# nanoshimarobot/dynamic_direct_lidar_odometry

Measured on AMD Instinct MI355X. Metric: GICP iters/sec + ms/scan, 131k-pt source → 500k-pt submap; pose Δ vs CPU ref, higher is better.
Workload: dtype f32 search / f64 normal equations; 1 GPU; cfg3 S2M GICP: 131,072-pt 64x2048 scan -> 500,000-pt 4-keyframe submap, LM, maxCorr 2.0 m, maxIter 32, transEps 0.01; target_points=500000, parallelism=replicas x1

## Files before the change

dynamic_direct_lidar_odometry_amd/__init__.py:

```python
from __future__ import annotations

import ctypes as C
import math
import os
import sys

import numpy as np

__all__ = ["GicpParams", "GicpResult", "Context", "NanoGICP", "GicpError", "lib_path", "load", "s2s_batch",
           "REG_NONE", "REG_MIN_EIG", "REG_NORMALIZED_MIN_EIG", "REG_PLANE", "REG_FROBENIUS",
           "GAUSS_NEWTON", "LEVENBERG_MARQUARDT", "SOURCE", "TARGET"]

REG_NONE, REG_MIN_EIG, REG_NORMALIZED_MIN_EIG, REG_PLANE, REG_FROBENIUS = range(5)
GAUSS_NEWTON, LEVENBERG_MARQUARDT = 0, 1
SOURCE, TARGET = 0, 1
COV_MAT4D, COV_SYM6 = 0, 1

_HERE = os.path.dirname(os.path.abspath(__file__))
_LIB = None

STATUS = {0: "GICP_OK", 1: "GICP_EINVAL", 2: "GICP_ENOTARGET", 3: "GICP_ENOSOURCE", 4: "GICP_ETOOFEW",
          5: "GICP_EHIP", 6: "GICP_ENOMEM", 7: "GICP_ESTATE", 8: "GICP_ENONFINITE", 9: "GICP_ECOMM"}


# ... 153 lines not shown
        "gicp_get_tie_order": (I, [P, C.POINTER(C.c_int)]),
        "gicp_set_option": (I, [P, I, I]),
        "gicp_get_option": (I, [P, I, C.POINTER(C.c_int)]),
        "gicp_set_default_option": (I, [I, I]),
        "gicp_get_default_option": (I, [I, C.POINTER(C.c_int)]),
        "gicp_tie_builder_set": (I, [P, P, C.c_size_t, C.c_size_t]),
        "gicp_tie_builder_export": (I, [P, P, C.c_size_t, C.POINTER(C.c_void_p), C.POINTER(C.c_size_t)]),
        "gicp_set_tie_tree": (I, [P, P, C.c_size_t]),
        "gicp_set_tie_trees_from_root": (I, [P, I, P, P]),
        "gicp_get_device_bytes": (I, [P, C.POINTER(C.c_int64), I]),
        "gicp_debug_nftree": (I, [P, I, P, P, P, S, C.POINTER(S)]),
        "gicp_debug_nfbuild": (I, [P, I, I, P, P, P, P, S]),
        "gicp_set_target_grid": (I, [P, I]),
        "gicp_get_target_grid_info": (I, [P, C.POINTER(GicpGridInfo)]),
        "gicp_get_lookup_stats": (I, [P, C.POINTER(C.c_int64)]),
    }
    for name, (res, args) in sig.items():
        f = getattr(L, name)
        f.restype = res
        f.argtypes = args
    _LIB = L
    return L


def default_params(**kw) -> GicpParams:
    p = GicpParams()
    load().gicp_default_params(C.byref(p))
    for k, v in kw.items():
        setattr(p, k, v)
    return p


def _ptr(a):
# ... 227 lines not shown
        return idx, d

    def set_target_grid(self, mode=GRID_AUTO):
        self._check(self.L.gicp_set_target_grid(self.h, int(mode)))

    def grid_info(self) -> dict:
        info = GicpGridInfo()
        self._check(self.L.gicp_get_target_grid_info(self.h, C.byref(info)))
        return info.as_dict()

    def lookup_walk_groups(self) -> int:
        v = C.c_int64(0)
        self._check(self.L.gicp_get_lookup_stats(self.h, C.byref(v)))
        return int(v.value)

    def set_tie_order(self, nanoflann_order=True):
        self._check(self.L.gicp_set_tie_order(self.h, 1 if nanoflann_order else 0))

    def nftree(self, side):
        nn = C.c_size_t(0)
        self._check(self.L.gicp_debug_nftree(self.h, side, None, None, None, 0, C.byref(nn)))
        n = self.size(side)
        vind = np.empty(n, np.int32)
        nodes = np.empty((nn.value, 4), np.int32)
        div = np.empty((nn.value, 2), np.float32)
        self._check(self.L.gicp_debug_nftree(self.h, side, _ptr(vind), _ptr(nodes), _ptr(div), nn.value, C.byref(nn)))
        return vind, nodes, div

    def nfbuild_debug(self, side, stop=-1, scratch_bytes=1 << 20):
        n = self.size(side)
# ... 184 lines not shown
```

dynamic_direct_lidar_odometry_amd/csrc/capi.hip:

```cpp
#include <hip/hip_runtime.h>

#include <atomic>
#include <thread>

#include <hipcub/hipcub.hpp>
#include <rccl/rccl.h>

#include <dlfcn.h>

#include <algorithm>
#include <cfloat>
#include <cmath>
#include <cstdio>
#include <cstdlib>
#include <cstring>
#include <limits>
#include <map>
#include <memory>
#include <mutex>
#include <string>
#include <tuple>
#include <thread>
#include <vector>

// ... 453 lines not shown
    none->info.build_status = s;
    t.grid = none;
    g_last_error.clear();
    return GICP_OK;
  }
  t.grid = g;
  return GICP_OK;
}

struct JobCommit {
  gicp_ctx* c;
  bool ok = false;
  explicit JobCommit(gicp_ctx* ctx) : c(ctx) {}
  void done() { ok = true; }
  ~JobCommit() {
    if (!ok) c->job_last_valid = false;
  }
};

void finalize_job(gicp_ctx* c) {
  AlignJob& j = *c->job_host;
  j.job_full = 0;
  AlignJob probe = j;
  std::memcpy(probe.guess_R, c->job_last.guess_R, sizeof(probe.guess_R));
  std::memcpy(probe.guess_t, c->job_last.guess_t, sizeof(probe.guess_t));
  probe.job_full = c->job_last.job_full;
  probe.ticket = c->job_last.ticket;
  if (!c->job_last_valid || std::memcmp(&probe, &c->job_last, sizeof(AlignJob)) != 0) {
    j.job_full = 1;
    c->job_last = j;
    c->job_last_valid = true;
// ... 208 lines not shown
void drop_set(GraphSet& gs) {
  for (auto& p : gs.first) drop_pair(p);
  gs.first.clear();
  drop_pair(gs.rest[0]);
  drop_pair(gs.rest[1]);
  gs.key.fill(-1);
}

void drop_graphs(gicp_ctx* c) {
  for (auto& gs : c->gsets) drop_set(gs);
  c->gsets.clear();
}

gicp_status graph_set(gicp_ctx* c, const std::array<long long, 7>& key, int nblocks, GraphSet** out);

gicp_status run_align_graph(gicp_ctx* c, int max_it, int nblocks, int* final_chunk) {
  const void* jd = c->job_dev.p;
  const LinGeom g = geometry(c);
  (void)nblocks;
  const std::array<long long, 7> key{{(long long)(uintptr_t)c->slab.p | (c->comm ? 1 : 0), (long long)(uintptr_t)jd,
                                      g.seed_blocks, g.scan_blocks, g.mom_blocks, g.lds_boxes,
                                      g.grid ? (g.grid_walk ? 2L : 1L) * g.lookup_blocks : 0}};
  const bool use_graph = !c->comm || c->comm_graphs;
  const int first = c->params.fixed_iterations > 0
                        ? std::max(1, std::min(max_it, kMaxFixedChunk))
                        : std::max(1, std::min({c->predicted_iters, max_it, kMaxFirstChunk}));
  GraphSet* gs = nullptr;
  if (use_graph) {
    gicp_status s = graph_set(c, key, nblocks, &gs);
    if (s) {
      drop_graphs(c);
      (void)hipGetLastError();
      if (!c->comm) return s;
      c->comm_graphs = false;
      return run_align_graph(c, max_it, nblocks, final_chunk);
    }
  }
  if (use_graph && !gs->first[first - 1].ge) {
    gicp_status s = capture_chunk(c, true, first, nblocks, 0, &gs->first[first - 1]);
    if (s) {
      drop_graphs(c);
      return s;
    }
  }
  auto launch_chunk = [&](int k) -> gicp_status {
    const bool is_first = k == 0;
    if (use_graph) {
      HIP_TRY(hipGraphLaunch(is_first ? gs->first[first - 1].ge : gs->rest[k & 1].ge, c->stream));
      return GICP_OK;
    }
    return enqueue_chunk(c, is_first, is_first ? first : 1, nblocks, k & 1);
  };
  const int nchunks = 1 + (max_it - first);
  while ((int)c->chunk_ev.size() < nchunks) {
    hipEvent_t e;
    HIP_TRY(hipEventCreateWithFlags(&e, hipEventDisableTiming));
    c->chunk_ev.push_back(e);
  }
  gicp_status s = launch_chunk(0);
  if (s) return s;
  HIP_TRY(hipEventRecord(c->chunk_ev[0], c->stream));
// ... 366 lines not shown
  c->tie_tree.reset();
  invalidate_align(c);
  return GICP_OK;
}

gicp_status gicp_share_source(gicp_ctx* dst, const gicp_ctx* src) {
  if (!dst || !src) return fail(GICP_EINVAL, "null ctx");
  if (dst->device != src->device) return fail(GICP_EINVAL, "contexts live on different devices");
  dst->src = src->src;
  invalidate_align(dst);
  return GICP_OK;
}

gicp_status gicp_align(gicp_ctx* c, const float* guess16, float* out16, gicp_result* res) {
  if (!c) return fail(GICP_EINVAL, "null ctx");
  begin_ties(c);
  gicp_status s = set_device(c);
  if (s) return s;
  s = maybe_build_grid(c);
  if (s) return s;
  s = prepare_align(c);
  if (s) return s;
  const int ns = c->src.cloud->n;
  const int nblocks = linearize_blocks(ns);
  hipEvent_t end_ev = c->ev1;
  int reruns = 0;
  for (;;) {
    s = fill_job(c, guess16, nblocks);
    if (s) return s;
    finalize_job(c);
    JobCommit commit(c);
    const int max_it = c->job_host->max_iterations;
    end_ev = c->ev1;
    if (c->profiling) HIP_TRY(hipEventRecord(c->ev0, c->stream));
    if (c->profiling || max_it <= 0) {
      s = max_it > 0 ? run_align_eager_profiled(c, max_it, nblocks) : GICP_OK;
      if (s) return s;
      if (max_it <= 0) launch_align_init(c->stream, c->job_dev.as<AlignJob>(), c->job_host_dev);
      HIP_TRY(hipGetLastError());
      commit.done();
      HIP_TRY(hipEventRecord(c->ev1, c->stream));
      HIP_TRY(hipMemcpyAsync(c->state_host, c->state_dev.p, sizeof(AlignState), hipMemcpyDeviceToHost, c->stream));
      HIP_TRY(hipStreamSynchronize(c->stream));
      c->state_slot = 0;
      c->tail_pending = false;
    } else {
      int fc = 0;
      s = run_align_graph(c, max_it, nblocks, &fc);
      if (s) return s;
      commit.done();
      end_ev = c->chunk_ev[fc];
    }
    if (!final_state(c).tie_pending || reruns > 0) break;
    s = ensure_tie_tree(c);
    if (s) return s;
    ++reruns;
  }
  const AlignState& st = final_state(c);
  c->have_align = st.iter > 0;
  c->last_nsrc = ns;
  if (out16) {
    for (int r = 0; r < 3; ++r) {
      for (int cc = 0; cc < 3; ++cc) out16[4 * r + cc] = (float)st.R[3 * r + cc];
      out16[4 * r + 3] = (float)st.t[r];
    }
// ... 21 lines not shown
      double tot = 0.0;
      for (int i = 0; i < st.iter; ++i) {
        float m = 0.f;
        HIP_TRY(hipEventElapsedTime(&m, c->prof_ev[2 * i], c->prof_ev[2 * i + 1]));
        tot += m;
      }
      res->linearize_ms = tot;
    }
  }
  s = check_ties(c);
  if (s) return s;
  if (st.tie_err || st.tie_pending)
    return fail(GICP_EHIP, "nanoflann tie order: a tied correspondence could not be re-run (bits " +
                               std::to_string(st.tie_err) + (st.tie_pending ? ", no tree" : "") + ")");
  if (st.lm_failed) g_last_error = "lm not converged!!";
  return GICP_OK;
}

gicp_status gicp_get_residuals(gicp_ctx* c, double* out, size_t n) {
  if (!c || !out) return fail(GICP_EINVAL, "null argument");
  if (!c->have_align || !c->src.cloud || !c->tgt.cloud) return fail(GICP_ESTATE, "no linearization to report residuals of");
  if ((int)n != c->src.cloud->n) return fail(GICP_EINVAL, "n != source size");
  gicp_status s = set_device(c);
  if (s) return s;
  HIP_TRY(c->tmp_out.ensure(sizeof(double) * n));
  launch_residuals(c->stream, c->job_dev.as<AlignJob>(), (int)n, c->tmp_out.as<double>());
  HIP_TRY(hipGetLastError());
  if (c->comm)
    NCCL_TRY(rccl().all_reduce(c->tmp_out.p, c->tmp_out.p, n, ncclFloat64, ncclMin, c->comm, c->stream));
  HIP_TRY(hipMemcpyAsync(out, c->tmp_out.p, sizeof(double) * n, hipMemcpyDeviceToHost, c->stream));
// ... 66 lines not shown
  const size_t bytes = (n - 1) * stride + 12;
  HIP_TRY(c->tmp_out.ensure(bytes + 256));
  float* dT = reinterpret_cast<float*>(c->tmp_out.as<char>() + ((bytes + 63) / 64) * 64);
  HIP_TRY(hipMemcpyAsync(dT, T, sizeof(T), hipMemcpyHostToDevice, c->stream));
  HIP_TRY(hipMemcpyAsync(c->tmp_out.p, out_xyz, bytes, hipMemcpyHostToDevice, c->stream));
  launch_transform(c->stream, c->src.cloud->pts.as<float4>(), (int)n, c->src.cloud->perm.as<int>(), dT,
                   c->tmp_out.as<float>(), stride / 4);
  HIP_TRY(hipGetLastError());
  HIP_TRY(hipMemcpyAsync(out_xyz, c->tmp_out.p, bytes, hipMemcpyDeviceToHost, c->stream));
  HIP_TRY(hipStreamSynchronize(c->stream));
  return GICP_OK;
}

gicp_status gicp_linearize(gicp_ctx* c, const double* pose16, double* H36, double* b6, double* cost, int32_t* ncorr) {
  if (!c || !pose16) return fail(GICP_EINVAL, "null argument");
  begin_ties(c);
  gicp_status s = set_device(c);
  if (s) return s;
  s = maybe_build_grid(c);
  if (s) return s;
  s = prepare_align(c);
  if (s) return s;
  const int ns = c->src.cloud->n;
  const int nblocks = linearize_blocks(ns);
  for (int rerun = 0;; ++rerun) {
    float g[16];
    for (int i = 0; i < 16; ++i) g[i] = 0.f;
    s = fill_job(c, g, nblocks);
    if (s) return s;
    for (int r = 0; r < 3; ++r) {
// ... 167 lines not shown
}

gicp_status gicp_set_target_grid(gicp_ctx* c, int mode) {
  if (!c) return fail(GICP_EINVAL, "null ctx");
  if (mode < GICP_GRID_OFF || mode > GICP_GRID_ON) return fail(GICP_EINVAL, "grid mode must be 0 (off), 1 (auto) or 2 (on)");
  c->grid_mode = mode;
  return GICP_OK;
}

gicp_status gicp_get_target_grid_info(gicp_ctx* c, gicp_grid_info* out) {
  if (!c || !out) return fail(GICP_EINVAL, "null argument");
  std::memset(out, 0, sizeof(*out));
  if (!c->tgt.cloud || !c->tgt.cloud->grid) return GICP_OK;
  *out = c->tgt.cloud->grid->info;
  out->built = grid_active(c) ? 1 : 0;
  return GICP_OK;
}

gicp_status gicp_get_lookup_stats(gicp_ctx* c, int64_t* walk_groups) {
  if (!c || !walk_groups) return fail(GICP_EINVAL, "null argument");
  *walk_groups = -1;
  if (!c->fb.p || !c->src.cloud) return GICP_OK;
  gicp_status s = set_device(c);
  if (s) return s;
  unsigned v = 0;
  const FbLayout fl(c->src.cloud->n);
  HIP_TRY(hipMemcpyAsync(&v, c->fb.as<char>() + fl.ctr + sizeof(unsigned) * kFbSegs * 32, sizeof(unsigned),
                         hipMemcpyDeviceToHost, c->stream));
  HIP_TRY(hipStreamSynchronize(c->stream));
  *walk_groups = v;
// ... 580 lines not shown
```

dynamic_direct_lidar_odometry_amd/csrc/gicp_types.hpp:

```cpp
#pragma once
#include <stdint.h>

namespace ddlo {

constexpr int kLeafSize = 32;
constexpr int kFanout = 64;
constexpr int kMaxLevels = 5;
constexpr int kDirBits = 18;
constexpr int kFineBits = 6;
constexpr int kFineMin = 32;
__host__ __device__ constexpr long fine_dir_ints(int n) {
  return (1L << kDirBits) + 2 + (1L << kDirBits) + ((long)(n / (kFineMin + 1) + 1) << kFineBits) / 2;
}

constexpr int kMoments = 74;
constexpr int kMomentSlots = 96;
constexpr int kSlabStride = 80;
constexpr int kStatFields = 8;

constexpr int kTaskRegions = 64;
constexpr int kCtrStride = 32;
constexpr int kTasksPerGroup = 48;

struct CloudDev {
// ... 153 lines not shown
  unsigned long long* key2;
  int tie_detect;
  int tie_ab;
  int tie_scan;
  const int* tgt_nf_status;
  NfTreeDev tgt_nf;
  int grid_on;
  CellGridDev grid;
  unsigned* fb_count;
  int* fb_list;
  int fb_seg_cap;
  unsigned short* fb_mask;
};
constexpr int kFbSegs = 8;

constexpr int kNfMaxLevels = 40;
constexpr int kNfLevelSpare = 2;

struct NfCtl {
  int nnodes, nsmall, err;
  int nchunks[2];
  int ntask[kNfMaxLevels + 1];
  int dbg[16];
};

struct NfTask {
  int node, begin, count, chunk0;
  float lo[3], hi[3];
  unsigned mm[6];
  int feat;
// ... 57 lines not shown
```

dynamic_direct_lidar_odometry_amd/csrc/launch.hpp:

```cpp
#pragma once
#include <hip/hip_runtime.h>

#include "gicp_types.hpp"

namespace ddlo {

void launch_pack_bbox(hipStream_t s, const unsigned char* raw, size_t stride, int n, float4* out, float* partial,
                      int* nonfinite, int nblocks);
void launch_bbox_final(hipStream_t s, const float* partial, int nparts, float* quant);
void launch_morton(hipStream_t s, const float4* pts, int n, const float* quant, unsigned long long* keys, int* vals);
void launch_gather(hipStream_t s, const float4* raw, const int* perm, int n, int npad, float4* sorted, int* inv_perm);
void launch_key_dir(hipStream_t s, const unsigned long long* keys, int n, int* dir);
void launch_leaf_soa_boxes(hipStream_t s, const float4* pts, int n, int nleaves, float* soa, float4* lo, float4* hi);
void launch_level_boxes(hipStream_t s, const float4* clo, const float4* chi, int nchild, int nparent, float4* plo,
                        float4* phi);
struct TieList {
  int* list;
  int* count;
  int cap = 0;
  __device__ __forceinline__ void push(int i) const {
    const int slot = atomicAdd(count, 1);
    if (slot < cap) list[slot] = i;
  }
};
// ... 7 lines not shown
void launch_cov_export(hipStream_t s, const double* cov6, int layout, int n, const int* perm, double* out);
size_t tie_prune_scratch_bytes(int n, int cap);
hipError_t launch_tie_prune(hipStream_t s, const NfTreeDev& t, int cap, const int* local_index, int n_local,
                            void* scratch, NfNode* out_nodes, float4* out_pts, unsigned* counts);
void launch_align_init(hipStream_t s, AlignJob* job, const AlignJob* job_src);
struct LinGeom {
  int seed_blocks, scan_blocks, mom_blocks, lds_boxes, lookup_blocks;
  bool fuse_lm = false;
  AlignState* state = nullptr;
  bool grid = false;
  bool grid_walk = true;
};
bool lm_fusion_enabled(bool lookup);
LinGeom linearize_geometry(int nsrc, int tgt_upper);
void launch_linearize(hipStream_t s, const AlignJob* job, const LinGeom& g, AlignState* publish = nullptr);
int search_queries_per_wave();
int task_cap_per_region(int nsrc);
int moment_blocks(int nsrc);
int lm_slab_rows_max();
void launch_lm_step(hipStream_t s, const AlignJob* job, AlignState* st, const double* slab, int nblocks,
                    const double* premom, AlignState* publish);
void launch_mom_reduce(hipStream_t s, const AlignJob* job);
void launch_residuals(hipStream_t s, const AlignJob* job, int nsrc, double* out);
void launch_residual_image(hipStream_t s, const float4* pts, const int* perm, const int* inv_perm, int n,
                           const double* residual, double tmin, double tmax, int W, int H, int* winner, float* img,
                           float* xyz);
void launch_transform(hipStream_t s, const float4* pts, int n, const int* perm, const float* T16, float* out,
                      size_t stride_floats);
void launch_export_corr(hipStream_t s, const AlignJob* job, int nsrc, int* corr, float* sqd);

// ... 37 lines not shown
```

dynamic_direct_lidar_odometry_amd/csrc/lm_step.hpp:

```cpp
#pragma once
#include <hip/hip_runtime.h>

#include "gicp_types.hpp"
#include "search.hpp"

namespace ddlo {

static __device__ void so3_exp_d(const double w[3], double R[9]) {
  const double theta_sq = w[0] * w[0] + w[1] * w[1] + w[2] * w[2];
  double imag, real;
  if (theta_sq < 1e-10) {
    const double theta_quad = theta_sq * theta_sq;
    imag = 0.5 - 1.0 / 48.0 * theta_sq + 1.0 / 3840.0 * theta_quad;
    real = 1.0 - 1.0 / 8.0 * theta_sq + 1.0 / 384.0 * theta_quad;
  } else {
    const double theta = sqrt(theta_sq);
    const double half = 0.5 * theta;
    double sh, ch;
    sincos(half, &sh, &ch);
    imag = sh / theta;
    real = ch;
  }
  const double qw = real, qx = imag * w[0], qy = imag * w[1], qz = imag * w[2];
  const double tx = 2 * qx, ty = 2 * qy, tz = 2 * qz;
// ... 202 lines not shown
  if (tid < kSlabStride) {
    double s = 0.0;
#pragma unroll
    for (int p = 0; p < kLmParts; ++p) s += part[p][tid];
    mom[tid] = s;
  }
}

#ifdef DDLO_LM_PROF
#define LM_PROF(i) if (threadIdx.x == 0) lm_t[i] = __builtin_amdgcn_s_memtime()
#define LM_PROF_TRIAL(i) if (threadIdx.x == 0) lm_tt[i] = __builtin_amdgcn_s_memtime()
#else
#define LM_PROF(i)
#define LM_PROF_TRIAL(i)
#endif
template <bool PREMOM>
__device__ __forceinline__ void lm_step_body(const AlignJob* __restrict__ job, AlignState* __restrict__ st,
                                             const double* __restrict__ slab, int nblocks,
                                             const double* __restrict__ premom) {
#ifdef DDLO_LM_PROF
  unsigned long long lm_t[6], lm_tt[4] = {0, 0, 0, 0};
#endif
  LM_PROF(0);
  __shared__ double part[kLmParts][kSlabStride];
  __shared__ double mom[kSlabStride];
  __shared__ double nq[kNeqEntries];
  double* const Hs = nq;
  double* const bs = nq + 36;
  double* const W12 = nq + 42;
  double* const g12 = nq + 186;
  __shared__ double tr_lambda[kMaxTrials], tr_cm[kMaxTrials], tr_fro[kMaxTrials];
  __shared__ double tr_R[kMaxTrials][9], tr_t[kMaxTrials][3];
  __shared__ double tr_d[kMaxTrials][12], tr_row[kMaxTrials][12], tr_den[kMaxTrials], tr_x[kMaxTrials][6];
  __shared__ double Rt_s[12];
  __shared__ int tr_conv[kMaxTrials];
  const int tid = threadIdx.x;
  const int it_pre = st->iter;
  const int trials_pre = st->lm_trials;
  const int rec_pre = st->rec;
  const float src_radius = st->src_radius;
  const double lambda_pre = st->lambda;
  double rt_v = 0.0;
  if (tid < 12) rt_v = tid < 9 ? st->R[tid] : st->t[tid - 9];
  const int optimizer = job->optimizer, lm_max_iterations = job->lm_max_iterations;
  const int fixed_iterations = job->fixed_iterations, max_iterations = job->max_iterations;
  const double lm_init_lambda_factor = job->lm_init_lambda_factor;
  const double rotation_epsilon = job->rotation_epsilon, transformation_epsilon = job->transformation_epsilon;
  const int reuse = job->reuse;
  const float reuse_rec_eps = job->reuse_rec_eps, reuse_rec_conv = job->reuse_rec_conv;
  NeqTerm E{};
  if (tid < kNeqEntries) E = kNeq.e[tid];
  if constexpr (PREMOM) {
    if (tid < kSlabStride) mom[tid] = gp(premom)[tid];
  } else {
    reduce_slab(slab, nblocks, part, mom);
  }
  if (tid < 12) Rt_s[tid] = rt_v;
  __syncthreads();
// ... 90 lines not shown
    ok = ball != 0ull;
    chosen = ok ? (int)__builtin_ctzll(ball) : ntr - 1;
    const double rho_c = __shfl(rho, chosen);
    accept = ok && !(rho_c < 0);
    if (lane == 0) {
      st->lm_trials = trials_pre + (ok ? chosen + 1 : ntr);
      if (accept) {
        const double c = 2 * rho_c - 1;
        st->lambda = tr_lambda[chosen] * fmax(1.0 / 3.0, 1 - c * c * c);
      } else if (ok) {
        st->lambda = tr_lambda[chosen];
      } else {
        st->lambda = tr_lambda[ntr - 1] * 2.0;
      }
    }
  }
  if (lane == 0) {
    st->nr_iterations = it_pre;
    st->final_cost = mom[kMomY0];
    st->num_corr = (int)mom[kMomCount];
    if (rec_pre) st->any_rec = 1;
    st->iter = it_pre + 1;
    st->have_prev = 1;
    int done = 0;
    if (!ok) {
      st->lm_failed = 1;
      done = 1;
    } else if (tr_conv[chosen]) {
      st->converged = 1;
      done = 1;
    }
    if (it_pre + 1 >= max_iterations) done = 1;
    if (done) st->done = 1;
  }
  double v = 0.0;
  if (accept) {
    const double* Rd = tr_R[chosen];
    if (lane < 9) {
      const int i = lane / 3, j = lane % 3;
      v = Rd[3 * i + 0] * Rt_s[0 + j] + Rd[3 * i + 1] * Rt_s[3 + j] + Rd[3 * i + 2] * Rt_s[6 + j];
      st->R[lane] = v;
    } else if (lane < 12) {
      const int i = lane - 9;
      v = (Rd[3 * i + 0] * Rt_s[9] + Rd[3 * i + 1] * Rt_s[10] + Rd[3 * i + 2] * Rt_s[11]) + tr_t[chosen][i];
      st->t[i] = v;
    } else if (lane >= 16 && lane < 16 + 36) {
      st->final_hessian[lane - 16] = Hs[lane - 16];
    }
  }
  int rec = reuse;
  if (accept) {
    const double tn0 = __shfl(v, 9), tn1 = __shfl(v, 10), tn2 = __shfl(v, 11);
    const double* dt = tr_t[chosen];
    const double mv = sqrt(tr_fro[chosen]) * ((double)src_radius + sqrt(tn0 * tn0 + tn1 * tn1 + tn2 * tn2)) +
                      sqrt(dt[0] * dt[0] + dt[1] * dt[1] + dt[2] * dt[2]);
    rec = rec && mv < (double)reuse_rec_eps && (fixed_iterations > 0 || tr_cm[chosen] > (double)reuse_rec_conv);
  }
  if (lane == 0) st->rec = rec;
  LM_PROF(5);
#ifdef DDLO_LM_PROF
  if (tid == 0)
    printf("lm_prof %d %llu %llu %llu %llu %llu %llu %llu %llu %llu\n", it_pre, lm_t[1] - lm_t[0], lm_t[2] - lm_t[1],
           lm_t[3] - lm_t[2], lm_t[4] - lm_t[3], lm_t[5] - lm_t[4], lm_tt[0] - lm_t[2], lm_tt[1] - lm_tt[0],
// ... 6 lines not shown
```

dynamic_direct_lidar_odometry_amd/csrc/moments.hip:

```cpp
#include <hip/hip_runtime.h>

#include <cstddef>

#include "gicp_types.hpp"
#include "search.hpp"
#include "nftree.hpp"
#include "cov_math.hpp"
#include "launch.hpp"
#include "launch_util.hpp"
#include "linearize_internal.hpp"
#include "lm_step.hpp"

namespace ddlo {

struct Contrib {
  double M[6];
  double q[3];
  double qq[6];
  double v[3];
  double y;
  double c;
};

template <int S>
// ... 193 lines not shown
  int pending, resolved, err;
};
constexpr int kTieThread = 64 * (kMomWaves - 1);
__device__ __forceinline__ TieWords fetch_tie_words(AlignState* st) {
  TieWords tw{0, 0, 0};
  __hip_atomic_compare_exchange_strong(&st->tie_pending, &tw.pending, 0, __ATOMIC_RELAXED, __ATOMIC_RELAXED,
                                       __HIP_MEMORY_SCOPE_AGENT);
  __hip_atomic_compare_exchange_strong(&st->ties_resolved, &tw.resolved, 0, __ATOMIC_RELAXED, __ATOMIC_RELAXED,
                                       __HIP_MEMORY_SCOPE_AGENT);
  __hip_atomic_compare_exchange_strong(&st->tie_err, &tw.err, 0, __ATOMIC_RELAXED, __ATOMIC_RELAXED,
                                       __HIP_MEMORY_SCOPE_AGENT);
  return tw;
}

__device__ __forceinline__ void publish_state(const AlignJob* __restrict__ job, AlignState* __restrict__ st,
                                              AlignState* __restrict__ publish, const TieWords& tw) {
  static_assert(sizeof(AlignState) % 8 == 0, "AlignState is copied in 8-byte words");
  static_assert(offsetof(AlignState, pub) == sizeof(AlignState) - 8, "the publication word is the last 8 bytes");
  static_assert(offsetof(AlignState, iter) % 8 == 0 && offsetof(AlignState, done) == offsetof(AlignState, iter) + 4,
                "iter and done are one 8-byte word");
  __shared__ int tie_s[3];
  if (threadIdx.x == kTieThread) {
    tie_s[0] = tw.pending;
    tie_s[1] = tw.resolved;
    tie_s[2] = tw.err;
  }
  asm volatile("s_waitcnt vmcnt(0)" ::: "memory");
  __syncthreads();
  const auto src = gpw(reinterpret_cast<unsigned long long*>(st));
  const auto dst = gpw(reinterpret_cast<unsigned long long*>(publish));
  constexpr int kWords = (int)(sizeof(AlignState) / 8);
// ... 1 lines not shown
  auto patch = [](unsigned long long v, int w, size_t off, int val) {
    if ((size_t)w != off / 8) return v;
    const int sh = (int)(off & 4) * 8;
    return (v & ~(0xffffffffull << sh)) | ((unsigned long long)(unsigned)val << sh);
  };
  __shared__ unsigned long long iter_s;
  const int w = threadIdx.x;
  if (w < kWords) {
    unsigned long long v = __hip_atomic_load(src + w, __ATOMIC_RELAXED, __HIP_MEMORY_SCOPE_AGENT);
    v = patch(v, w, offsetof(AlignState, tie_pending), tie_s[0]);
    v = patch(v, w, offsetof(AlignState, ties_resolved), tie_s[1]);
    v = patch(v, w, offsetof(AlignState, tie_err), tie_s[2]);
    dst[w] = v;
    if (w == (int)(offsetof(AlignState, iter) / 8)) iter_s = v;
  }
  const unsigned long long tk = job->ticket;
  asm volatile("s_waitcnt vmcnt(0)" ::: "memory");
  __syncthreads();
  if (threadIdx.x == 0) {
    const unsigned long long id = iter_s;
    const unsigned long long w = (tk << 17) | ((unsigned long long)((unsigned)(id >> 32) != 0u) << 16) | (id & 0xffffu);
    __hip_atomic_store(&publish->pub, w, __ATOMIC_RELEASE, __HIP_MEMORY_SCOPE_SYSTEM);
  }
}

template <bool FUSE_LM, bool LOOKUP = false>
__global__ __launch_bounds__(64 * kMomWaves) void k_moments(const AlignJob* __restrict__ job,
                                                            AlignState* __restrict__ st, AlignState* __restrict__ publish) {
#ifdef DDLO_MOM_PROF
  unsigned long long mp_t[kMomProfWords] = {0, 0, 0, 0, 0, 0, 0};
#endif
  MOM_PROF(0);
  const auto sg = gp(st);
  double R[9], t[3];
  for (int e = 0; e < 9; ++e) R[e] = sg->R[e];
  for (int e = 0; e < 3; ++e) t[e] = sg->t[e];
  const int st_rec = sg->rec, st_any_rec = sg->any_rec;
  if (__builtin_amdgcn_readfirstlane(sg->done)) {
    if (FUSE_LM && publish && blockIdx.x == 0) {
      TieWords tw{};
      if (threadIdx.x == kTieThread) tw = fetch_tie_words(st);
      publish_state(job, st, publish, tw);
    }
    return;
  }
  const CloudDev src = job->src;
  const CloudDev tgt = job->tgt;
  const auto src_cov = gp(job->src_cov);
  const auto tgt_cov = gp(job->tgt_cov);
  const auto key = gp((const unsigned long long*)job->key);
  const auto corr = gpw(job->corr);
  const auto sqd = gpw(job->sqd);
  const auto slab = gpw(job->slab);
  const double max_corr2 = job->max_corr2;
  const int rec = st_rec;
  const int first_rec_done = st_any_rec;
  const int tie_detect = job->tie_detect;
  const bool slice_check = tie_detect && job->tie_scan >= 2 && !(job->tie_ab & 4);
  const bool tie3m = tie_detect && job->tie_scan == 3 && !rec;
  __shared__ NfWaveStack tie_stk[kMomWaves];
  const int lane = lane_id();
  const int wib = threadIdx.x >> 6;
#ifdef DDLO_MOM_PROF
  __builtin_amdgcn_s_waitcnt(0);
#endif
  MOM_PROF(1);
  const int wave = blockIdx.x * kMomWaves + wib;
  const int nwaves_total = gridDim.x * kMomWaves;
  const int ngroups = (src.n + 63) >> 6;
  if (blockIdx.x == 0 && threadIdx.x < kTaskRegions) job->task_ctr[threadIdx.x * kCtrStride] = 0u;
  if (blockIdx.x == 0 && job->grid_on && threadIdx.x == 0) {
    unsigned t = 0;
    for (int sg = 0; sg < kFbSegs; ++sg) t += job->fb_count[sg * 32];
    job->fb_count[kFbSegs * 32] += t;
    for (int sg = 0; sg < kFbSegs; ++sg) job->fb_count[sg * 32] = 0u;
  }
  double acc0 = 0.0, acc1 = 0.0, acc2 = 0.0;
  for (int g = wave; g < ngroups; g += nwaves_total) {
    const int i = g * 64 + lane;
    const bool active = i < src.n;
    int j = -1;
    unsigned kj = 0xffffffffu;
    float kd = INFINITY;
    bool tied = false;
    float4 a = make_float4(0.f, 0.f, 0.f, 0.f), b = a;
    double ca[6] = {0, 0, 0, 0, 0, 0}, cb[6] = {0, 0, 0, 0, 0, 0};
    float lqx = 0.f, lqy = 0.f, lqz = 0.f;
    unsigned long long lkey = 0ull;
    unsigned lsec = 0xffffffffu;
// ... 233 lines not shown
    __shared__ int last_s;
    asm volatile("s_waitcnt vmcnt(0)" ::: "memory");
    __syncthreads();
    unsigned* const arrive = job->task_ctr + kTaskRegions * kCtrStride;
    if (threadIdx.x == 0) last_s = atomicAdd(arrive, 1u) == gridDim.x - 1;
    __syncthreads();
    if (!last_s) return;
    if (threadIdx.x == 0) {
      __builtin_amdgcn_fence(__ATOMIC_ACQUIRE, "agent");
      asm volatile("s_waitcnt vmcnt(0)" ::: "memory");
      atomicExch(arrive, 0u);
    }
    __syncthreads();
    TieWords tw{};
    if (publish && threadIdx.x == kTieThread) tw = fetch_tie_words(st);
    lm_step_body<false>(job, st, job->slab, job->nblocks, nullptr);
    if (publish) publish_state(job, st, publish, tw);
  }
}
template __global__ void k_moments<false>(const AlignJob*, AlignState*, AlignState*);
template __global__ void k_moments<true>(const AlignJob*, AlignState*, AlignState*);
template __global__ void k_moments<false, true>(const AlignJob*, AlignState*, AlignState*);
template __global__ void k_moments<true, true>(const AlignJob*, AlignState*, AlignState*);

__global__ __launch_bounds__(kLmThreads) void k_mom_reduce(const AlignJob* __restrict__ job) {
  AlignState* st = job->state;
  if (__builtin_amdgcn_readfirstlane(st->done)) return;
  __shared__ double part[kLmParts][kSlabStride];
  __shared__ double mom[kSlabStride];
  reduce_slab(job->slab, job->nblocks, part, mom);
  __syncthreads();
  if (threadIdx.x < kSlabStride) gpw(job->mom)[threadIdx.x] = mom[threadIdx.x];
}

__global__ __launch_bounds__(kLmThreads) void k_lm_step(const AlignJob* __restrict__ job, AlignState* __restrict__ st,
                                                        const double* __restrict__ slab, int nblocks,
                                                        const double* __restrict__ premom,
                                                        AlignState* __restrict__ publish) {
  TieWords tw{};
  if (publish && threadIdx.x == kTieThread) tw = fetch_tie_words(st);
  if (!__builtin_amdgcn_readfirstlane(st->done)) {
    if (premom) lm_step_body<true>(job, st, slab, nblocks, premom);
    else lm_step_body<false>(job, st, slab, nblocks, nullptr);
  }
  if (publish) publish_state(job, st, publish, tw);
}

void launch_linearize(hipStream_t s, const AlignJob* job, const LinGeom& g, AlignState* publish) {
  static const int fused_lookup = env_knob("DDLO_GRID_FUSED", 1);
  if (g.grid && !g.grid_walk && fused_lookup) {
    if (g.fuse_lm) k_moments<true, true><<<g.mom_blocks, 64 * kMomWaves, 0, s>>>(job, g.state, publish);
    else k_moments<false, true><<<g.mom_blocks, 64 * kMomWaves, 0, s>>>(job, g.state, nullptr);
    return;
  }
  if (g.grid) launch_cell_lookup(s, job, g);
  if (!g.grid || g.grid_walk) launch_nn_walk(s, job, g);
  if (g.fuse_lm) k_moments<true><<<g.mom_blocks, 64 * kMomWaves, 0, s>>>(job, g.state, publish);
  else k_moments<false><<<g.mom_blocks, 64 * kMomWaves, 0, s>>>(job, g.state, nullptr);
}
int moment_blocks(int nsrc) {
  const int groups = (nsrc + 63) / 64;
  return std::max(1, std::min((groups + kMomWaves - 1) / kMomWaves, kMomBlocksMax));
}
int lm_slab_rows_max() { return kMomBlocksMax; }
void launch_lm_step(hipStream_t s, const AlignJob* job, AlignState* st, const double* slab, int nblocks,
                    const double* premom, AlignState* publish) {
  k_lm_step<<<1, kLmThreads, 0, s>>>(job, st, slab, nblocks, premom, publish);
}
void launch_mom_reduce(hipStream_t s, const AlignJob* job) { k_mom_reduce<<<1, kLmThreads, 0, s>>>(job); }

}

#ifdef DDLO_MOM_PROF
extern "C" int ddlo_dev_mom_prof(unsigned long long* out) {
// ... 4 lines not shown
```

dynamic_direct_lidar_odometry_amd/csrc/runtime.hpp:

```cpp
#pragma once
#include <hip/hip_runtime.h>

#include <hipcub/hipcub.hpp>
#include <rccl/rccl.h>

#include <array>
#include <cfloat>
#include <cmath>
#include <cstring>
#include <map>
#include <memory>
#include <mutex>
#include <string>
#include <tuple>
#include <vector>

#include "../../include/ddlo_gicp.h"
#include "gicp_types.hpp"
#include "launch.hpp"
#include "devknobs.hpp"

#define HIP_TRY(expr)                                                                       \
  do {                                                                                      \
    hipError_t _e = (expr);                                                                 \
// ... 296 lines not shown
constexpr int kNfGraphs = 4;

constexpr int kDefaultPredictedIters = 4;

struct gicp_ctx {
  int device = 0;
  hipStream_t stream = nullptr;
  gicp_params params{};
  Side src, tgt;
  DevBuf raw_bytes, raw_pts, partial, nonfinite, keys_tmp, vals_tmp, sort_tmp, knn;
  DevBuf corr, sqd, slab, job_dev, state_dev, tmp_out, stats;
  bool stats_on = false;
  AlignJob* job_host = nullptr;
  AlignJob job_last{};
  bool job_last_valid = false;
  AlignJob* job_host_dev = nullptr;
  AlignState* state_host_dev = nullptr;
  AlignState* state_host = nullptr;
  int state_slot = 0;
  hipEvent_t tail_ev = nullptr;
  bool tail_pending = false;
  int grid_max_mb = 0;
  unsigned long long ticket = 0;
  int* flag_host = nullptr;
  bool have_align = false;
  int last_nsrc = 0;
  std::vector<GraphSet> gsets;
  long long graph_clock = 0;
  int predicted_iters = kDefaultPredictedIters;
  std::vector<hipEvent_t> chunk_ev;
// ... 532 lines not shown
          for (int p : pos) std::fprintf(f, " %d", p < side.cloud->n ? perm[p] : -1);
          std::fprintf(f, "\n");
          std::fclose(f);
        }
      }
    }
  }
  HIP_TRY(hipGetLastError());
  side.cov = cv;
  return GICP_OK;
}

inline void invalidate_align(gicp_ctx* c) {
  c->have_align = false;
  c->job_last_valid = false;
}

}
}
```

include/ddlo_gicp.h:

```cpp
#ifndef DDLO_GICP_H
#define DDLO_GICP_H

#include <stddef.h>
#include <stdint.h>

#ifdef __cplusplus
extern "C" {
#endif

#define DDLO_GICP_ABI_VERSION 4

typedef enum gicp_status {
  GICP_OK = 0,
  GICP_EINVAL = 1,
  GICP_ENOTARGET = 2,
  GICP_ENOSOURCE = 3,
  GICP_ETOOFEW = 4,
  GICP_EHIP = 5,
  GICP_ENOMEM = 6,
  GICP_ESTATE = 7,
  GICP_ENONFINITE = 8,
  GICP_ECOMM = 9
} gicp_status;

// ... 103 lines not shown
  int64_t bytes;
  int64_t coarse_cells;
  int64_t band_cells;
  int64_t nomatch_cells;
  int64_t overflow_cells;
  int64_t level_cells[4];
  int64_t fine_cells;
  int64_t fallback_fine;
  int64_t entries;
  int64_t uses_walk;
  int64_t build_status;
  int64_t scratch_bytes;
} gicp_grid_info;
gicp_status gicp_get_target_grid_info(struct gicp_ctx* ctx, gicp_grid_info* out);
gicp_status gicp_get_lookup_stats(struct gicp_ctx* ctx, int64_t* walk_groups);

gicp_status gicp_debug_nftree(struct gicp_ctx* ctx, int side, int32_t* vind, int32_t* nodes4, float* div2, size_t cap,
                              size_t* nnodes);
gicp_status gicp_debug_nfbuild(struct gicp_ctx* ctx, int side, int stop, int32_t* vind, int64_t* info16,
                               int32_t* status2, void* scratch, size_t scratch_cap);
gicp_status gicp_get_moments(const struct gicp_ctx* ctx, double* out80);
typedef struct gicp_lm_state {
  double R[9];
  double t[3];
  double lambda;
  double final_cost;
  double final_hessian[36];
  double last_b[6];
  double last_mom[80];
  int32_t iter;
// ... 45 lines not shown
```

Measured before the change: 32930 GICP iters/s.

## Add fresh-start first iteration kernel that skips job upload and state init

When the previous align completed cleanly via the graph path and only the guess pose/ticket changed, the first chunk launches a dedicated fused moments+LM kernel. That kernel takes the initial pose by value, writes the job header on device, and resets LM state itself. This is meant to avoid the per-align init/state-reset and job-copy work ahead of the first iteration and the first-chunk graph launch. It adds a special-case code path with its own state reset logic that must exactly mirror the normal init, so there is a risk of stale state.

```diff
diff --git a/dynamic_direct_lidar_odometry_amd/__init__.py b/dynamic_direct_lidar_odometry_amd/__init__.py
--- a/dynamic_direct_lidar_odometry_amd/__init__.py
+++ b/dynamic_direct_lidar_odometry_amd/__init__.py
@@ -191,9 +191,14 @@
         "gicp_set_target_grid": (I, [P, I]),
         "gicp_get_target_grid_info": (I, [P, C.POINTER(GicpGridInfo)]),
         "gicp_get_lookup_stats": (I, [P, C.POINTER(C.c_int64)]),
+        "gicp_get_start_counts": (I, [P, C.POINTER(C.c_int64), C.POINTER(C.c_int64)]),
     }
     for name, (res, args) in sig.items():
-        f = getattr(L, name)
+        f = getattr(L, name, None)
+        if f is None and name == "gicp_get_start_counts" and "DDLO_GICP_LIB" in os.environ:
+            continue
+        if f is None:
+            raise AttributeError(f"{path}: no symbol {name}")
         f.restype = res
         f.argtypes = args
     _LIB = L
@@ -451,6 +456,11 @@
         self._check(self.L.gicp_get_lookup_stats(self.h, C.byref(v)))
         return int(v.value)
 
+    def start_counts(self):
+        f, i = C.c_int64(0), C.c_int64(0)
+        self._check(self.L.gicp_get_start_counts(self.h, C.byref(f), C.byref(i)))
+        return int(f.value), int(i.value)
+
     def set_tie_order(self, nanoflann_order=True):
         self._check(self.L.gicp_set_tie_order(self.h, 1 if nanoflann_order else 0))
 
diff --git a/dynamic_direct_lidar_odometry_amd/csrc/capi.hip b/dynamic_direct_lidar_odometry_amd/csrc/capi.hip
--- a/dynamic_direct_lidar_odometry_amd/csrc/capi.hip
+++ b/dynamic_direct_lidar_odometry_amd/csrc/capi.hip
@@ -491,7 +491,7 @@
   explicit JobCommit(gicp_ctx* ctx) : c(ctx) {}
   void done() { ok = true; }
   ~JobCommit() {
-    if (!ok) c->job_last_valid = false;
+    if (!ok) c->job_last_valid = c->fresh_ok = false;
   }
 };
 
@@ -730,7 +730,22 @@
 
 gicp_status graph_set(gicp_ctx* c, const std::array<long long, 7>& key, int nblocks, GraphSet** out);
 
-gicp_status run_align_graph(gicp_ctx* c, int max_it, int nblocks, int* final_chunk) {
+bool fresh_start_enabled() {
+  static const bool on = [] {
+    const char* v = dev_getenv("DDLO_FRESH_START");
+    return !(v && *v == '0');
+  }();
+  return on;
+}
+
+bool fresh_start_allowed(const gicp_ctx* c, bool prev_ok, int max_it) {
+  if (!prev_ok || !fresh_start_enabled() || c->job_host->job_full != 0 || max_it <= 0) return false;
+  if (c->comm || c->profiling || c->stats_on) return false;
+  const LinGeom g = geometry(c);
+  return linearize_is_one_kernel(g) && g.fuse_lm;
+}
+
+gicp_status run_align_graph(gicp_ctx* c, int max_it, int nblocks, bool fresh, int* final_chunk) {
   const void* jd = c->job_dev.p;
   const LinGeom g = geometry(c);
   (void)nblocks;
@@ -749,10 +764,10 @@
       (void)hipGetLastError();
       if (!c->comm) return s;
       c->comm_graphs = false;
-      return run_align_graph(c, max_it, nblocks, final_chunk);
-    }
-  }
-  if (use_graph && !gs->first[first - 1].ge) {
+      return run_align_graph(c, max_it, nblocks, fresh, final_chunk);
+    }
+  }
+  if (use_graph && !fresh && !gs->first[first - 1].ge) {
     gicp_status s = capture_chunk(c, true, first, nblocks, 0, &gs->first[first - 1]);
     if (s) {
       drop_graphs(c);
@@ -761,6 +776,18 @@
   }
   auto launch_chunk = [&](int k) -> gicp_status {
     const bool is_first = k == 0;
+    if (is_first && fresh) {
+      const AlignJob& jh = *c->job_host;
+      FreshStart fs{};
+      std::memcpy(fs.R, jh.guess_R, sizeof(fs.R));
+      std::memcpy(fs.t, jh.guess_t, sizeof(fs.t));
+      fs.ticket = jh.ticket;
+      fs.job_w = c->job_dev.as<AlignJob>();
+      fs.rec0 = jh.reuse && jh.reuse_rec0;
+      launch_linearize_fresh(c->stream, c->job_dev.as<AlignJob>(), g, fs, first == 1 ? c->state_host_dev : nullptr);
+      HIP_TRY(hipGetLastError());
+      return first > 1 ? enqueue_chunk(c, false, first - 1, nblocks, 0) : GICP_OK;
+    }
     if (use_graph) {
       HIP_TRY(hipGraphLaunch(is_first ? gs->first[first - 1].ge : gs->rest[k & 1].ge, c->stream));
       return GICP_OK;
@@ -1157,6 +1184,9 @@
 
 gicp_status gicp_align(gicp_ctx* c, const float* guess16, float* out16, gicp_result* res) {
   if (!c) return fail(GICP_EINVAL, "null ctx");
+  bool prev_ok = c->fresh_ok;
+  c->fresh_ok = false;
+  bool graph_path = false;
   begin_ties(c);
   gicp_status s = set_device(c);
   if (s) return s;
@@ -1174,6 +1204,9 @@
     finalize_job(c);
     JobCommit commit(c);
     const int max_it = c->job_host->max_iterations;
+    const bool fresh = fresh_start_allowed(c, prev_ok, max_it);
+    prev_ok = false;
+    ++(fresh ? c->fresh_aligns : c->init_aligns);
     end_ev = c->ev1;
     if (c->profiling) HIP_TRY(hipEventRecord(c->ev0, c->stream));
     if (c->profiling || max_it <= 0) {
@@ -1187,11 +1220,13 @@
       HIP_TRY(hipStreamSynchronize(c->stream));
       c->state_slot = 0;
       c->tail_pending = false;
+      graph_path = false;
     } else {
       int fc = 0;
-      s = run_align_graph(c, max_it, nblocks, &fc);
+      s = run_align_graph(c, max_it, nblocks, fresh, &fc);
       if (s) return s;
       commit.done();
+      graph_path = true;
       end_ev = c->chunk_ev[fc];
     }
     if (!final_state(c).tie_pending || reruns > 0) break;
@@ -1243,6 +1278,7 @@
     return fail(GICP_EHIP, "nanoflann tie order: a tied correspondence could not be re-run (bits " +
                                std::to_string(st.tie_err) + (st.tie_pending ? ", no tree" : "") + ")");
   if (st.lm_failed) g_last_error = "lm not converged!!";
+  c->fresh_ok = graph_path && !st.tie_pending && !st.ties_resolved && !st.tie_err;
   return GICP_OK;
 }
 
@@ -1339,6 +1375,7 @@
 
 gicp_status gicp_linearize(gicp_ctx* c, const double* pose16, double* H36, double* b6, double* cost, int32_t* ncorr) {
   if (!c || !pose16) return fail(GICP_EINVAL, "null argument");
+  c->fresh_ok = false;
   begin_ties(c);
   gicp_status s = set_device(c);
   if (s) return s;
@@ -1536,6 +1573,13 @@
   if (!c->tgt.cloud || !c->tgt.cloud->grid) return GICP_OK;
   *out = c->tgt.cloud->grid->info;
   out->built = grid_active(c) ? 1 : 0;
+  return GICP_OK;
+}
+
+gicp_status gicp_get_start_counts(gicp_ctx* c, int64_t* fresh_starts, int64_t* init_starts) {
+  if (!c) return fail(GICP_EINVAL, "null ctx");
+  if (fresh_starts) *fresh_starts = c->fresh_aligns;
+  if (init_starts) *init_starts = c->init_aligns;
   return GICP_OK;
 }
 
diff --git a/dynamic_direct_lidar_odometry_amd/csrc/gicp_types.hpp b/dynamic_direct_lidar_odometry_amd/csrc/gicp_types.hpp
--- a/dynamic_direct_lidar_odometry_amd/csrc/gicp_types.hpp
+++ b/dynamic_direct_lidar_odometry_amd/csrc/gicp_types.hpp
@@ -191,6 +191,14 @@
 };
 constexpr int kFbSegs = 8;
 
+struct FreshStart {
+  double R[9];
+  double t[3];
+  unsigned long long ticket;
+  AlignJob* job_w;
+  int rec0;
+};
+
 constexpr int kNfMaxLevels = 40;
 constexpr int kNfLevelSpare = 2;
 
diff --git a/dynamic_direct_lidar_odometry_amd/csrc/launch.hpp b/dynamic_direct_lidar_odometry_amd/csrc/launch.hpp
--- a/dynamic_direct_lidar_odometry_amd/csrc/launch.hpp
+++ b/dynamic_direct_lidar_odometry_amd/csrc/launch.hpp
@@ -45,6 +45,9 @@
 bool lm_fusion_enabled(bool lookup);
 LinGeom linearize_geometry(int nsrc, int tgt_upper);
 void launch_linearize(hipStream_t s, const AlignJob* job, const LinGeom& g, AlignState* publish = nullptr);
+bool linearize_is_one_kernel(const LinGeom& g);
+void launch_linearize_fresh(hipStream_t s, const AlignJob* job, const LinGeom& g, const FreshStart& fs,
+                            AlignState* publish = nullptr);
 int search_queries_per_wave();
 int task_cap_per_region(int nsrc);
 int moment_blocks(int nsrc);
diff --git a/dynamic_direct_lidar_odometry_amd/csrc/lm_step.hpp b/dynamic_direct_lidar_odometry_amd/csrc/lm_step.hpp
--- a/dynamic_direct_lidar_odometry_amd/csrc/lm_step.hpp
+++ b/dynamic_direct_lidar_odometry_amd/csrc/lm_step.hpp
@@ -240,10 +240,10 @@
 #define LM_PROF(i)
 #define LM_PROF_TRIAL(i)
 #endif
-template <bool PREMOM>
+template <bool PREMOM, bool FRESH = false>
 __device__ __forceinline__ void lm_step_body(const AlignJob* __restrict__ job, AlignState* __restrict__ st,
                                              const double* __restrict__ slab, int nblocks,
-                                             const double* __restrict__ premom) {
+                                             const double* __restrict__ premom, const FreshStart* fs = nullptr) {
 #ifdef DDLO_LM_PROF
   unsigned long long lm_t[6], lm_tt[4] = {0, 0, 0, 0};
 #endif
@@ -261,13 +261,19 @@
   __shared__ double Rt_s[12];
   __shared__ int tr_conv[kMaxTrials];
   const int tid = threadIdx.x;
-  const int it_pre = st->iter;
-  const int trials_pre = st->lm_trials;
-  const int rec_pre = st->rec;
+  const int it_pre = FRESH ? 0 : st->iter;
+  const int trials_pre = FRESH ? 0 : st->lm_trials;
+  const int rec_pre = FRESH ? fs->rec0 : st->rec;
   const float src_radius = st->src_radius;
-  const double lambda_pre = st->lambda;
+  const double lambda_pre = FRESH ? -1.0 : st->lambda;
   double rt_v = 0.0;
-  if (tid < 12) rt_v = tid < 9 ? st->R[tid] : st->t[tid - 9];
+  if constexpr (FRESH) {
+#pragma unroll
+    for (int e = 0; e < 12; ++e)
+      if (tid == e) rt_v = e < 9 ? fs->R[e] : fs->t[e - 9];
+  } else {
+    if (tid < 12) rt_v = tid < 9 ? st->R[tid] : st->t[tid - 9];
+  }
   const int optimizer = job->optimizer, lm_max_iterations = job->lm_max_iterations;
   const int fixed_iterations = job->fixed_iterations, max_iterations = job->max_iterations;
   const double lm_init_lambda_factor = job->lm_init_lambda_factor;
@@ -388,24 +394,37 @@
         st->lambda = tr_lambda[ntr - 1] * 2.0;
       }
     }
+  } else if (FRESH && lane == 0) {
+    st->lm_trials = 0;
+    st->lambda = -1.0;
   }
   if (lane == 0) {
     st->nr_iterations = it_pre;
     st->final_cost = mom[kMomY0];
     st->num_corr = (int)mom[kMomCount];
     if (rec_pre) st->any_rec = 1;
+    else if (FRESH) st->any_rec = 0;
     st->iter = it_pre + 1;
     st->have_prev = 1;
     int done = 0;
-    if (!ok) {
-      st->lm_failed = 1;
-      done = 1;
-    } else if (tr_conv[chosen]) {
-      st->converged = 1;
-      done = 1;
-    }
-    if (it_pre + 1 >= max_iterations) done = 1;
-    if (done) st->done = 1;
+    if constexpr (FRESH) {
+      const int failed = !ok, conv = ok && tr_conv[chosen];
+      st->lm_failed = failed;
+      st->converged = conv;
+      done = failed | conv;
+      if (it_pre + 1 >= max_iterations) done = 1;
+      st->done = done;
+    } else {
+      if (!ok) {
+        st->lm_failed = 1;
+        done = 1;
+      } else if (tr_conv[chosen]) {
+        st->converged = 1;
+        done = 1;
+      }
+      if (it_pre + 1 >= max_iterations) done = 1;
+      if (done) st->done = 1;
+    }
   }
   double v = 0.0;
   if (accept) {
@@ -421,6 +440,9 @@
     } else if (lane >= 16 && lane < 16 + 36) {
       st->final_hessian[lane - 16] = Hs[lane - 16];
     }
+  } else if (FRESH && lane < 12) {
+    if (lane < 9) st->R[lane] = Rt_s[lane];
+    else st->t[lane - 9] = Rt_s[lane];
   }
   int rec = reuse;
   if (accept) {
diff --git a/dynamic_direct_lidar_odometry_amd/csrc/moments.hip b/dynamic_direct_lidar_odometry_amd/csrc/moments.hip
--- a/dynamic_direct_lidar_odometry_amd/csrc/moments.hip
+++ b/dynamic_direct_lidar_odometry_amd/csrc/moments.hip
@@ -231,7 +231,8 @@
 }
 
 __device__ __forceinline__ void publish_state(const AlignJob* __restrict__ job, AlignState* __restrict__ st,
-                                              AlignState* __restrict__ publish, const TieWords& tw) {
+                                              AlignState* __restrict__ publish, const TieWords& tw,
+                                              const unsigned long long* ticket = nullptr) {
   static_assert(sizeof(AlignState) % 8 == 0, "AlignState is copied in 8-byte words");
   static_assert(offsetof(AlignState, pub) == sizeof(AlignState) - 8, "the publication word is the last 8 bytes");
   static_assert(offsetof(AlignState, iter) % 8 == 0 && offsetof(AlignState, done) == offsetof(AlignState, iter) + 4,
@@ -263,7 +264,7 @@
     dst[w] = v;
     if (w == (int)(offsetof(AlignState, iter) / 8)) iter_s = v;
   }
-  const unsigned long long tk = job->ticket;
+  const unsigned long long tk = ticket ? *ticket : job->ticket;
   asm volatile("s_waitcnt vmcnt(0)" ::: "memory");
   __syncthreads();
   if (threadIdx.x == 0) {
@@ -273,25 +274,46 @@
   }
 }
 
-template <bool FUSE_LM, bool LOOKUP = false>
-__global__ __launch_bounds__(64 * kMomWaves) void k_moments(const AlignJob* __restrict__ job,
-                                                            AlignState* __restrict__ st, AlignState* __restrict__ publish) {
+template <bool FUSE_LM, bool LOOKUP, bool FRESH>
+__device__ __forceinline__ void moments_body(const AlignJob* __restrict__ job, AlignState* __restrict__ st,
+                                             AlignState* __restrict__ publish, const FreshStart* fs) {
+  static_assert(!FRESH || (FUSE_LM && LOOKUP), "the fresh start exists for the fused one-kernel lookup iteration only");
 #ifdef DDLO_MOM_PROF
   unsigned long long mp_t[kMomProfWords] = {0, 0, 0, 0, 0, 0, 0};
 #endif
   MOM_PROF(0);
-  const auto sg = gp(st);
   double R[9], t[3];
-  for (int e = 0; e < 9; ++e) R[e] = sg->R[e];
-  for (int e = 0; e < 3; ++e) t[e] = sg->t[e];
-  const int st_rec = sg->rec, st_any_rec = sg->any_rec;
-  if (__builtin_amdgcn_readfirstlane(sg->done)) {
-    if (FUSE_LM && publish && blockIdx.x == 0) {
-      TieWords tw{};
-      if (threadIdx.x == kTieThread) tw = fetch_tie_words(st);
-      publish_state(job, st, publish, tw);
-    }
-    return;
+  int st_rec, st_any_rec;
+  if constexpr (FRESH) {
+    for (int e = 0; e < 9; ++e) R[e] = fs->R[e];
+    for (int e = 0; e < 3; ++e) t[e] = fs->t[e];
+    st_rec = fs->rec0;
+    st_any_rec = 0;
+    if (blockIdx.x == 0 && threadIdx.x == 64) {
+      static_assert(offsetof(AlignJob, guess_t) == offsetof(AlignJob, guess_R) + 72 &&
+                        offsetof(AlignJob, job_full) == offsetof(AlignJob, guess_R) + 96 &&
+                        offsetof(AlignJob, ticket) == offsetof(AlignJob, guess_R) + 104,
+                    "guess_R, guess_t, job_full, ticket: the job's 14 header words");
+      AlignJob* const jw = fs->job_w;
+      for (int e = 0; e < 9; ++e) jw->guess_R[e] = fs->R[e];
+      for (int e = 0; e < 3; ++e) jw->guess_t[e] = fs->t[e];
+      jw->job_full = 0;
+      jw->ticket = fs->ticket;
+    }
+  } else {
+    const auto sg = gp(st);
+    for (int e = 0; e < 9; ++e) R[e] = sg->R[e];
+    for (int e = 0; e < 3; ++e) t[e] = sg->t[e];
+    st_rec = sg->rec;
+    st_any_rec = sg->any_rec;
+    if (__builtin_amdgcn_readfirstlane(sg->done)) {
+      if (FUSE_LM && publish && blockIdx.x == 0) {
+        TieWords tw{};
+        if (threadIdx.x == kTieThread) tw = fetch_tie_words(st);
+        publish_state(job, st, publish, tw);
+      }
+      return;
+    }
   }
   const CloudDev src = job->src;
   const CloudDev tgt = job->tgt;
@@ -321,7 +343,8 @@
   if (blockIdx.x == 0 && job->grid_on && threadIdx.x == 0) {
     unsigned t = 0;
     for (int sg = 0; sg < kFbSegs; ++sg) t += job->fb_count[sg * 32];
-    job->fb_count[kFbSegs * 32] += t;
+    if constexpr (FRESH) job->fb_count[kFbSegs * 32] = 0u;
+    else job->fb_count[kFbSegs * 32] += t;
     for (int sg = 0; sg < kFbSegs; ++sg) job->fb_count[sg * 32] = 0u;
   }
   double acc0 = 0.0, acc1 = 0.0, acc2 = 0.0;
@@ -585,9 +608,20 @@
     __syncthreads();
     TieWords tw{};
     if (publish && threadIdx.x == kTieThread) tw = fetch_tie_words(st);
-    lm_step_body<false>(job, st, job->slab, job->nblocks, nullptr);
-    if (publish) publish_state(job, st, publish, tw);
-  }
+    lm_step_body<false, FRESH>(job, st, job->slab, job->nblocks, nullptr, fs);
+    if (publish) publish_state(job, st, publish, tw, FRESH ? &fs->ticket : nullptr);
+  }
+}
+
+template <bool FUSE_LM, bool LOOKUP = false>
+__global__ __launch_bounds__(64 * kMomWaves) void k_moments(const AlignJob* __restrict__ job,
+                                                            AlignState* __restrict__ st, AlignState* __restrict__ publish) {
+  moments_body<FUSE_LM, LOOKUP, false>(job, st, publish, nullptr);
+}
+__global__ __launch_bounds__(64 * kMomWaves) void k_moments_fresh(const AlignJob* __restrict__ job,
+                                                                  AlignState* __restrict__ st,
+                                                                  AlignState* __restrict__ publish, const FreshStart fs) {
+  moments_body<true, true, true>(job, st, publish, &fs);
 }
 template __global__ void k_moments<false>(const AlignJob*, AlignState*, AlignState*);
 template __global__ void k_moments<true>(const AlignJob*, AlignState*, AlignState*);
@@ -617,9 +651,12 @@
   if (publish) publish_state(job, st, publish, tw);
 }
 
+bool linearize_is_one_kernel(const LinGeom& g) {
+  static const int fused_lookup = env_knob("DDLO_GRID_FUSED", 1);
+  return g.grid && !g.grid_walk && fused_lookup;
+}
 void launch_linearize(hipStream_t s, const AlignJob* job, const LinGeom& g, AlignState* publish) {
-  static const int fused_lookup = env_knob("DDLO_GRID_FUSED", 1);
-  if (g.grid && !g.grid_walk && fused_lookup) {
+  if (linearize_is_one_kernel(g)) {
     if (g.fuse_lm) k_moments<true, true><<<g.mom_blocks, 64 * kMomWaves, 0, s>>>(job, g.state, publish);
     else k_moments<false, true><<<g.mom_blocks, 64 * kMomWaves, 0, s>>>(job, g.state, nullptr);
     return;
@@ -629,6 +666,10 @@
   if (g.fuse_lm) k_moments<true><<<g.mom_blocks, 64 * kMomWaves, 0, s>>>(job, g.state, publish);
   else k_moments<false><<<g.mom_blocks, 64 * kMomWaves, 0, s>>>(job, g.state, nullptr);
 }
+void launch_linearize_fresh(hipStream_t s, const AlignJob* job, const LinGeom& g, const FreshStart& fs,
+                            AlignState* publish) {
+  k_moments_fresh<<<g.mom_blocks, 64 * kMomWaves, 0, s>>>(job, g.state, publish, fs);
+}
 int moment_blocks(int nsrc) {
   const int groups = (nsrc + 63) / 64;
   return std::max(1, std::min((groups + kMomWaves - 1) / kMomWaves, kMomBlocksMax));
diff --git a/dynamic_direct_lidar_odometry_amd/csrc/runtime.hpp b/dynamic_direct_lidar_odometry_amd/csrc/runtime.hpp
--- a/dynamic_direct_lidar_odometry_amd/csrc/runtime.hpp
+++ b/dynamic_direct_lidar_odometry_amd/csrc/runtime.hpp
@@ -334,6 +334,8 @@
   AlignJob* job_host = nullptr;
   AlignJob job_last{};
   bool job_last_valid = false;
+  bool fresh_ok = false;
+  long long fresh_aligns = 0, init_aligns = 0;
   AlignJob* job_host_dev = nullptr;
   AlignState* state_host_dev = nullptr;
   AlignState* state_host = nullptr;
@@ -896,7 +898,8 @@
 inline void invalidate_align(gicp_ctx* c) {
   c->have_align = false;
   c->job_last_valid = false;
-}
-
-}
-}
+  c->fresh_ok = false;
+}
+
+}
+}
diff --git a/include/ddlo_gicp.h b/include/ddlo_gicp.h
--- a/include/ddlo_gicp.h
+++ b/include/ddlo_gicp.h
@@ -141,6 +141,7 @@
 } gicp_grid_info;
 gicp_status gicp_get_target_grid_info(struct gicp_ctx* ctx, gicp_grid_info* out);
 gicp_status gicp_get_lookup_stats(struct gicp_ctx* ctx, int64_t* walk_groups);
+gicp_status gicp_get_start_counts(struct gicp_ctx* ctx, int64_t* fresh_starts, int64_t* init_starts);
 
 gicp_status gicp_debug_nftree(struct gicp_ctx* ctx, int side, int32_t* vind, int32_t* nodes4, float* div2, size_t cap,
                               size_t* nnodes);
```

Result: faster. 35570 GICP iters/s, median of 6 (+8.0%).
